# ugadiarov-la-phystech-edu/OCRL

Hardware: AMD Instinct MI355X
Metric: images/sec (node) SLATE pretrain 128x128, 6 slots, 3 iters (higher is better)
Workload: dtype f32

## Files before the change

### include/ocrl_hip.h

```cpp
#ifndef OCRL_HIP_H
#define OCRL_HIP_H
#include <stddef.h>

#ifdef __cplusplus
extern "C" {
#endif

#define OCRL_ABI_VERSION 5

const char* ocrl_last_error(void);
int ocrl_abi_version(void);

typedef struct ocrl_slate ocrl_slate;
typedef struct ocrl_slate_config {
    int obs_size, obs_channels;
    int vocab_size, d_model;
    int cnn_hidden;
    int num_slots, num_iterations, slot_size, mlp_hidden;
    int num_dec_blocks, num_dec_heads;
    float dropout;
    int max_batch;
    int use_bcdec;
    int hard;
    int num_slot_heads;
// ... 80 lines not shown
int ocrl_conv2d_bwd_weight_ex(const ocrl_conv_wgrad_desc* d, float* ws, size_t ws_floats, void* stream);
size_t ocrl_conv2d_first_fwd_ws_floats(void);
int ocrl_conv2d_first_fwd(const float* obs, const float* w, const float* bias, float* y, int B, int H, int W, int relu, float* ws, size_t ws_floats,
                          void* stream);
size_t ocrl_conv2d_first_wgrad_ws_floats(int B, int H, int W);
int ocrl_conv2d_first_bwd_weight(const float* obs, const float* dy, float* dw, float* db, int B, int H, int W, int accumulate, float* ws, size_t ws_floats,
                                 void* stream);
int ocrl_layernorm_fwd(const float* x, const float* gamma, const float* beta, float* y, float* mean, float* rstd, long long R, int F, void* stream);
int ocrl_layernorm_bwd(const float* dy, const float* x, const float* mean, const float* rstd, const float* gamma, float* dx, float* dgb,
                       long long R, int F, float* ws, size_t ws_floats, void* stream);

int ocrl_sa_input_plan(long long R, int out[3]);
int ocrl_sa_input_fwd(const float* e4, const float* gamma, const float* beta, const float* W0, const float* b0, const float* W2, const float* b2,
                      float* mean, float* rstd, float* h1, float* x, long long R, int max_wgs, void* stream);
int ocrl_sa_input_bwd(const float* dx, const float* h1, const float* e4, const float* mean, const float* rstd, const float* gamma, const float* beta,
                      const float* W0, const float* W2, float* de4, float* dW0, float* db0, float* dW2, float* db2, float* dgamma, float* dbeta,
                      long long R, int max_wgs, float* ws, size_t ws_floats, void* stream);

int ocrl_attention_fwd(const float* q, const float* k, const float* v, float* o, float* lse, int B, int T, int d, int h, int ld,
                       float p, unsigned long long seed, unsigned site, void* stream);
int ocrl_attention_bwd(const float* q, const float* k, const float* v, const float* o, const float* lse, const float* dO,
                       float* dq, float* dk, float* dv, float* delta, int B, int T, int d, int h, int ld,
                       float p, unsigned long long seed, unsigned site, void* stream);

typedef struct ocrl_xattn_desc {
    const float* x; const float* resid; const float* mem;
    const float* Wq; const float* Wk; const float* Wv; const float* Wo;
    float* ck; float* cv; float* Ab; float* AbT; float* Vo; float* VoT; float* y; float* P;
    const float* gd;
    float* Pd; float* dS; float* dx; float* dAb; float* dVo; float* dck; float* dcv; float* dWq; float* dWo;
    float* pq; float* po; float* cs_ws; size_t cs_ws_floats;
    int B, T, K, d, h;
    float p; unsigned long long seed; unsigned site_p, site_o;
} ocrl_xattn_desc;
size_t ocrl_xattn_desc_size(void);
int ocrl_xattn_plan(int K, int d, int h, int out[5]);
int ocrl_xattn_fwd(const ocrl_xattn_desc* d, void* stream);
int ocrl_xattn_bwd(const ocrl_xattn_desc* d, void* stream);
int ocrl_cross_attn_fwd(const float* Q, const float* Km, const float* Vm, float* O, float* P, int B, int T, int K, int d, int h, float p,
                        unsigned long long seed, unsigned site, void* stream);
size_t ocrl_cross_attn_bwd_ws_floats(int B, int T, int K, int d, int h);
int ocrl_cross_attn_bwd(const float* dO, const float* Q, const float* Km, const float* Vm, const float* P, float* dQ, float* dKm, float* dVm,
                        int B, int T, int K, int d, int h, float p, unsigned long long seed, unsigned site, float* ws, size_t ws_floats,
                        void* stream);

int ocrl_obs_u8_to_f32(const unsigned char* obs_hwc, float* obs_chw, int B, int H, int W, int C, void* stream);
// ... 216 lines not shown
```

### ocrl_amd/_lib.py

```python
import ctypes
import os
from ctypes import POINTER, c_char_p, c_float, c_int, c_longlong, c_size_t, c_uint, c_ulonglong, c_void_p

_HERE = os.path.dirname(os.path.abspath(__file__))
LIB_PATH = os.environ.get("OCRL_HIP_LIB") or os.path.join(_HERE, "libocrl_hip.so")
_lib = None


class SlateConfig(ctypes.Structure):
    _fields_ = [(n, c_int) for n in ("obs_size", "obs_channels", "vocab_size", "d_model", "cnn_hidden", "num_slots",
                                      "num_iterations", "slot_size", "mlp_hidden", "num_dec_blocks", "num_dec_heads")] + \
               [("dropout", c_float), ("max_batch", c_int), ("use_bcdec", c_int), ("hard", c_int), ("num_slot_heads", c_int)]


class IodineConfig(ctypes.Structure):
    _fields_ = [(n, c_int) for n in ("obs_size", "obs_channels", "slot_size", "num_iterations", "num_slots")] + \
               [("sigma", c_float), ("beta", c_float), ("layer_norm", c_int), ("ref_mlp_hidden", c_int), ("max_batch", c_int)]


class GemmDesc(ctypes.Structure):
    _fields_ = [("A", c_void_p), ("B", c_void_p), ("C", c_void_p)] + \
               [(n, c_int) for n in ("M", "N", "K", "lda", "ldb", "ldc", "akc", "bkc", "batch", "batch_inner")] + \
               [(n, c_longlong) for n in ("sA", "sB", "sC", "sAi", "sBi", "sCi")] + \
               [("splitk", c_int), ("alpha", c_float), ("bias", c_void_p), ("relu", c_int),
# ... 144 lines not shown
    L.ocrl_conv2d_wgrad_ws_floats.argtypes = [c_int, c_int, c_int, c_int, c_int]
    L.ocrl_conv2d_wgrad_ws_floats.restype = c_size_t
    L.ocrl_conv2d_bwd_weight.argtypes = [p, p, p, p, c_int, c_int, c_int, c_int, c_int, c_int, p, c_size_t, p]
    L.ocrl_conv_desc_size.restype = c_size_t
    L.ocrl_conv_wgrad_desc_size.restype = c_size_t
    for name, cls in (("ocrl_conv_desc", ConvDesc), ("ocrl_conv_wgrad_desc", ConvWgradDesc)):
        n = getattr(L, name + "_size")()
        if n != ctypes.sizeof(cls):
            raise RuntimeError(f"libocrl_hip.so: {name} is {n} bytes, this binding's {cls.__name__} {ctypes.sizeof(cls)}")
    L.ocrl_conv2d_ex.argtypes = [POINTER(ConvDesc), p, c_size_t, p]
    L.ocrl_conv2d_bwd_weight_ex.argtypes = [POINTER(ConvWgradDesc), p, c_size_t, p]
    L.ocrl_conv2d_first_fwd_ws_floats.restype = c_size_t
    L.ocrl_conv2d_first_fwd.argtypes = [p, p, p, p, c_int, c_int, c_int, c_int, p, c_size_t, p]
    L.ocrl_conv2d_first_wgrad_ws_floats.argtypes = [c_int, c_int, c_int]
    L.ocrl_conv2d_first_wgrad_ws_floats.restype = c_size_t
    L.ocrl_conv2d_first_bwd_weight.argtypes = [p, p, p, p, c_int, c_int, c_int, c_int, p, c_size_t, p]
    L.ocrl_layernorm_fwd.argtypes = [p, p, p, p, p, p, c_longlong, c_int, p]
    L.ocrl_layernorm_bwd.argtypes = [p, p, p, p, p, p, p, c_longlong, c_int, p, c_size_t, p]
    L.ocrl_sa_input_plan.argtypes = [c_longlong, POINTER(c_int * 3)]
    L.ocrl_sa_input_fwd.argtypes = [p] * 11 + [c_longlong, c_int, p]
    L.ocrl_sa_input_bwd.argtypes = [p] * 16 + [c_longlong, c_int, p, c_size_t, p]
    L.ocrl_attention_fwd.argtypes = [p, p, p, p, p, c_int, c_int, c_int, c_int, c_int, c_float, c_ulonglong, c_uint, p]
    L.ocrl_attention_bwd.argtypes = [p, p, p, p, p, p, p, p, p, p, c_int, c_int, c_int, c_int, c_int, c_float, c_ulonglong, c_uint, p]
    L.ocrl_xattn_desc_size.restype = c_size_t
    if L.ocrl_xattn_desc_size() != ctypes.sizeof(XattnDesc):
        raise RuntimeError(f"libocrl_hip.so: ocrl_xattn_desc is {L.ocrl_xattn_desc_size()} bytes, this binding's XattnDesc {ctypes.sizeof(XattnDesc)}")
    L.ocrl_xattn_plan.argtypes = [c_int, c_int, c_int, POINTER(c_int * 5)]
    L.ocrl_xattn_fwd.argtypes = [POINTER(XattnDesc), p]
    L.ocrl_xattn_bwd.argtypes = [POINTER(XattnDesc), p]
    L.ocrl_cross_attn_fwd.argtypes = [p, p, p, p, p, c_int, c_int, c_int, c_int, c_int, c_float, c_ulonglong, c_uint, p]
    L.ocrl_cross_attn_bwd_ws_floats.argtypes = [c_int] * 5
    L.ocrl_cross_attn_bwd_ws_floats.restype = c_size_t
    L.ocrl_cross_attn_bwd.argtypes = [p] * 8 + [c_int] * 5 + [c_float, c_ulonglong, c_uint, p, c_size_t, p]
    L.ocrl_obs_u8_to_f32.argtypes = [p, p, c_int, c_int, c_int, c_int, p]
    L.ocrl_prof_enable.argtypes = [c_uint]
    L.ocrl_prof_collect.argtypes = [POINTER(ctypes.c_double * 8), POINTER(c_longlong * 8), c_int]
    L.ocrl_iodine_create.argtypes = [POINTER(IodineConfig), POINTER(p)]
    L.ocrl_iodine_destroy.argtypes = [p]
    L.ocrl_iodine_destroy.restype = None
    L.ocrl_iodine_param_count.argtypes = [p]
    L.ocrl_iodine_param_info.argtypes = [p, c_int, c_char_p, c_int, POINTER(c_int * 4), POINTER(c_int), POINTER(c_longlong), POINTER(c_longlong)]
    L.ocrl_iodine_flat_size.argtypes = [p]
    L.ocrl_iodine_flat_size.restype = c_longlong
    L.ocrl_iodine_workspace_bytes.argtypes = [p]
    L.ocrl_iodine_workspace_bytes.restype = c_size_t
    L.ocrl_iodine_bind.argtypes = [p, p, p, p, p, p, c_size_t]
# ... 125 lines not shown
```

### ocrl_amd/csrc/attention.hip

```cpp
#include "common.h"
#include "kernels.h"
#include <stdlib.h>

#define FA_BLK 64
#ifndef FA_LPT
#define FA_LPT 1
#endif
#ifndef FA_BWD_WGS
#define FA_BWD_WGS 3
#endif

typedef float f32x4_t __attribute__((ext_vector_type(4)));

template <int DH>
struct FaCfg {
    static constexpr int NC = DH / 16;
    static constexpr int LD = DH + 4;
};

template <int DH>
__device__ inline void fa_load_tile(float* s, const float* __restrict__ g, long long bt0, int row0, int T, int d, int hoff, float scale) {
    constexpr int F4 = DH / 4;
    constexpr int LD = FaCfg<DH>::LD;
    for (int idx = threadIdx.x; idx < FA_BLK * F4; idx += 256) {
// ... 174 lines not shown
    __shared__ float part[256];
    const int F4 = d >> 2, RPB = 256 / F4, HF = F4 / h;
    const int rl = threadIdx.x / F4, c4 = threadIdx.x - rl * F4;
    const long long row = (long long)blockIdx.x * RPB + rl;
    float s = 0.f;
    if (rl < RPB && row < BT) {
        const float4 x = *reinterpret_cast<const float4*>(dO + row * d + c4 * 4), y = *reinterpret_cast<const float4*>(O + row * d + c4 * 4);
        s = x.x * y.x + x.y * y.y + x.z * y.z + x.w * y.w;
    }
    part[threadIdx.x] = s;
    __syncthreads();
    if ((int)threadIdx.x < RPB * h) {
        const int r2 = threadIdx.x / h, hd = threadIdx.x - r2 * h;
        const long long row2 = (long long)blockIdx.x * RPB + r2;
        if (row2 < BT) {
            float t = 0.f;
            for (int k = 0; k < HF; ++k) t += part[r2 * F4 + hd * HF + k];
            const long long bb = row2 / T, q = row2 % T;
            delta[(bb * h + hd) * T + q] = t;
        }
    }
}

template <int DH>
__global__ __launch_bounds__(256, FA_BWD_WGS) void attn_bwd_kv_kernel(AttnArgs p) {
    constexpr int NC = FaCfg<DH>::NC, LD = FaCfg<DH>::LD;
    __shared__ __attribute__((aligned(16))) float Qs[FA_BLK * LD];
    __shared__ __attribute__((aligned(16))) float Gs[FA_BLK * LD];
    __shared__ float Ls[FA_BLK], Ds[FA_BLK];
    const int nkb = (p.T + FA_BLK - 1) / FA_BLK;
    int bid = blockIdx.x;
    const int nbh = gridDim.x / nkb;
    const int kb = FA_LPT ? bid / nbh : fa_block_index(bid % nkb, bid / nkb, nkb);
    bid = FA_LPT ? bid % nbh : bid / nkb;
    const int hd = bid % p.h;
    const long long b = bid / p.h;
    const int T = p.T, T4 = attn_drop_ld(p.T), d = p.ld, hoff = hd * DH;
    const long long bt0 = b * T;
    const int lane = threadIdx.x & 63, wv = threadIdx.x >> 6;
    const int li = lane & 15, g = lane >> 4;
    const int k_abs = kb * FA_BLK + wv * 16 + li;
    const float scale = rsqrtf((float)DH);
    const long long bh = b * p.h + hd;

    float4 kf[NC], vf[NC];
#pragma unroll
    for (int c = 0; c < NC; ++c) {
        kf[c] = make_float4(0.f, 0.f, 0.f, 0.f);
        vf[c] = kf[c];
        if (k_abs < T) {
            kf[c] = *reinterpret_cast<const float4*>(p.k + (bt0 + k_abs) * d + hoff + 16 * c + 4 * g);
            vf[c] = *reinterpret_cast<const float4*>(p.v + (bt0 + k_abs) * d + hoff + 16 * c + 4 * g);
        }
    }
    f32x4_t dk[NC], dv[NC];
#pragma unroll
    for (int c = 0; c < NC; ++c) { dk[c] = (f32x4_t){0.f, 0.f, 0.f, 0.f}; dv[c] = dk[c]; }
    const uint32_t thr = drop_thresh(p.p);
    const float dsc = p.p > 0.f ? 1.0f / (1.0f - p.p) : 1.f;

    float4 rq[FaRegs<DH>::N], rg[FaRegs<DH>::N];
    float rl = 0.f, rd = 0.f;
    auto fetch = [&](int qt) {
        fa_fetch<DH>(rq, p.q, bt0, qt * FA_BLK, T, d, hoff);
        fa_fetch<DH>(rg, p.dO, bt0, qt * FA_BLK, T, p.d, hoff);
        if (threadIdx.x < FA_BLK) {
            const int qq = qt * FA_BLK + threadIdx.x;
            rl = qq < T ? p.lse[bh * T + qq] : 0.f;
            rd = qq < T ? p.delta[bh * T + qq] : 0.f;
        }
    };
    fetch(kb);
    for (int qt = kb; qt < nkb; ++qt) {
        __syncthreads();
        fa_commit<DH>(Qs, rq, scale);
        fa_commit<DH>(Gs, rg, 1.f);
        if (threadIdx.x < FA_BLK) { Ls[threadIdx.x] = rl; Ds[threadIdx.x] = rd; }
        __syncthreads();
        if (qt + 1 < nkb) fetch(qt + 1);
#pragma unroll
        for (int sq = 0; sq < 4; ++sq) {
            f32x4_t s = (f32x4_t){0.f, 0.f, 0.f, 0.f}, dp = s;
#pragma unroll
            for (int c = 0; c < NC; ++c) {
                const float4 a = *reinterpret_cast<const float4*>(Qs + (16 * sq + li) * LD + 16 * c + 4 * g);
                s = MFMA16(a.x, kf[c].x, s);
                s = MFMA16(a.y, kf[c].y, s);
                s = MFMA16(a.z, kf[c].z, s);
                s = MFMA16(a.w, kf[c].w, s);
                const float4 e = *reinterpret_cast<const float4*>(Gs + (16 * sq + li) * LD + 16 * c + 4 * g);
                dp = MFMA16(e.x, vf[c].x, dp);
                dp = MFMA16(e.y, vf[c].y, dp);
                dp = MFMA16(e.z, vf[c].z, dp);
                dp = MFMA16(e.w, vf[c].w, dp);
            }
            uint2 hb = make_uint2(0u, 0u);
            if (p.p > 0.f) {
                const int qh = qt * FA_BLK + 16 * sq + 4 * g + (li & 3);
                const uint64_t idx = ((uint64_t)bh * T + (uint64_t)(qh < T ? qh : 0)) * T4 + (uint64_t)(k_abs < T4 ? k_abs : 0);
                hb = rng_bits4(p.seed, p.site, idx >> 2);
            }
            uint2 hq[4];
            hq[0] = make_uint2(__builtin_amdgcn_update_dpp(0, (int)hb.x, 0x00, 0xF, 0xF, false), __builtin_amdgcn_update_dpp(0, (int)hb.y, 0x00, 0xF, 0xF, false));
            hq[1] = make_uint2(__builtin_amdgcn_update_dpp(0, (int)hb.x, 0x55, 0xF, 0xF, false), __builtin_amdgcn_update_dpp(0, (int)hb.y, 0x55, 0xF, 0xF, false));
            hq[2] = make_uint2(__builtin_amdgcn_update_dpp(0, (int)hb.x, 0xAA, 0xF, 0xF, false), __builtin_amdgcn_update_dpp(0, (int)hb.y, 0xAA, 0xF, 0xF, false));
            hq[3] = make_uint2(__builtin_amdgcn_update_dpp(0, (int)hb.x, 0xFF, 0xF, 0xF, false), __builtin_amdgcn_update_dpp(0, (int)hb.y, 0xFF, 0xF, 0xF, false));
            f32x4_t pd, ds;
#pragma unroll
            for (int r = 0; r < 4; ++r) {
                const int ql = 16 * sq + 4 * g + r;
                const int qa = qt * FA_BLK + ql;
                float pr = 0.f;
                if (qa < T && k_abs <= qa && k_abs < T) pr = __expf(s[r] - Ls[ql]);
                float keep = 1.f;
                if (p.p > 0.f) keep = rng_keep(hq[r], li & 3, thr) ? dsc : 0.f;
                pd[r] = pr * keep;
                ds[r] = pr * (dp[r] * keep - Ds[ql]);
            }
            float ag[4][NC], aq[4][NC];
#pragma unroll
            for (int r = 0; r < 4; ++r)
#pragma unroll
                for (int c = 0; c < NC; ++c) {
                    ag[r][c] = Gs[(16 * sq + 4 * g + r) * LD + 16 * c + li];
                    aq[r][c] = Qs[(16 * sq + 4 * g + r) * LD + 16 * c + li];
                }
            __builtin_amdgcn_sched_barrier(0);
#pragma unroll
            for (int r = 0; r < 4; ++r)
#pragma unroll
                for (int c = 0; c < NC; ++c) {
                    dv[c] = MFMA16(ag[r][c], pd[r], dv[c]);
                    dk[c] = MFMA16(aq[r][c], ds[r], dk[c]);
                }
        }
    }
    if (k_abs < T) {
#pragma unroll
        for (int c = 0; c < NC; ++c) {
            *reinterpret_cast<float4*>(p.dv + (bt0 + k_abs) * d + hoff + 16 * c + 4 * g) = make_float4(dv[c][0], dv[c][1], dv[c][2], dv[c][3]);
// ... 69 lines not shown
#pragma unroll
            for (int st = 0; st < 4; ++st) { sS[st] = MFMA16(a[st].y, qf[c].y, sS[st]); sP[st] = MFMA16(e[st].y, gf[c].y, sP[st]); }
#pragma unroll
            for (int st = 0; st < 4; ++st) { sS[st] = MFMA16(a[st].z, qf[c].z, sS[st]); sP[st] = MFMA16(e[st].z, gf[c].z, sP[st]); }
#pragma unroll
            for (int st = 0; st < 4; ++st) { sS[st] = MFMA16(a[st].w, qf[c].w, sS[st]); sP[st] = MFMA16(e[st].w, gf[c].w, sP[st]); }
        }
#pragma unroll
        for (int st = 0; st < 4; ++st) {
            const int key0 = kt * FA_BLK + 16 * st + 4 * g;
            uint2 bits = make_uint2(0u, 0u);
            if (p.p > 0.f) {
                const uint64_t idx = ((uint64_t)bh * T + (uint64_t)(q_abs < T ? q_abs : 0)) * T4 + (uint64_t)key0;
                bits = rng_bits4(p.seed, p.site, idx >> 2);
            }
#pragma unroll
            for (int r = 0; r < 4; ++r) {
                float pr = 0.f;
                if (q_abs < T && key0 + r <= q_abs && key0 + r < T) pr = __expf(sS[st][r] - lse);
                float keep = 1.f;
                if (p.p > 0.f) keep = rng_keep(bits, r, thr) ? dsc : 0.f;
                sS[st][r] = pr * (sP[st][r] * keep - dlt);
            }
        }
        float ak[2][4][NC];
#pragma unroll
        for (int r = 0; r < 4; ++r)
#pragma unroll
            for (int c = 0; c < NC; ++c) ak[0][r][c] = Ks[(4 * g + r) * LD + 16 * c + li];
#pragma unroll
        for (int st = 0; st < 4; ++st) {
            if (st + 1 < 4) {
#pragma unroll
                for (int r = 0; r < 4; ++r)
#pragma unroll
                    for (int c = 0; c < NC; ++c) ak[(st + 1) & 1][r][c] = Ks[(16 * (st + 1) + 4 * g + r) * LD + 16 * c + li];
            }
            __builtin_amdgcn_sched_barrier(0);
#pragma unroll
            for (int r = 0; r < 4; ++r)
#pragma unroll
                for (int c = 0; c < NC; ++c) dq[c] = MFMA16(ak[st & 1][r][c], sS[st][r], dq[c]);
            __builtin_amdgcn_sched_barrier(0);
        }
    }
    if (q_abs < T) {
// ... 160 lines not shown
                        dst[16 * c] = first ? v : dst[16 * c] + v;
                    }
                }
            }
        }
        if (k_abs < T) {
#pragma unroll
            for (int c = 0; c < NC; ++c) {
                *reinterpret_cast<float4*>(p.dv + (bt0 + k_abs) * d + hoff + 16 * c + 4 * g) = make_float4(dv[c][0], dv[c][1], dv[c][2], dv[c][3]);
                *reinterpret_cast<float4*>(p.dk + (bt0 + k_abs) * d + hoff + 16 * c + 4 * g) = make_float4(dk[c][0], dk[c][1], dk[c][2], dk[c][3]);
            }
        }
    }
}

template <int DH>
static int attn_launch_dh(const AttnArgs& a, int mode, hipStream_t st) {
    const int nblk = cdiv(a.T, FA_BLK);
    const dim3 grid(a.B * a.h * nblk), blk(256);
    if (mode == 0) {
        hipLaunchKernelGGL((attn_fwd_kernel<DH>), grid, blk, 0, st, a);
        OCRL_CHECK_LAUNCH("attn_fwd");
    } else {
        const long long BT = (long long)a.B * a.T;
        OCRL_REQUIRE(a.d % 4 == 0 && a.d <= 1024 && (a.d / 4) % a.h == 0, "attention: d must be a multiple of 4*h, <= 1024");
        hipLaunchKernelGGL(attn_delta_kernel, dim3(cdiv(BT, 256 / (a.d / 4))), dim3(256), 0, st, a.dO, a.o, a.delta, BT, a.T, a.d, a.h);
        OCRL_CHECK_LAUNCH("attn_delta");
        const char* fe = getenv("OCRL_ATTN_BWD");
        if (fe && atoi(fe) == 1) {
            hipLaunchKernelGGL((attn_bwd_fused_kernel<DH>), dim3(a.B * a.h), dim3(512), 0, st, a);
            OCRL_CHECK_LAUNCH("attn_bwd_fused");
        } else {
        hipLaunchKernelGGL((attn_bwd_kv_kernel<DH>), grid, blk, 0, st, a);
        OCRL_CHECK_LAUNCH("attn_bwd_kv");
        hipLaunchKernelGGL((attn_bwd_q_kernel<DH>), grid, blk, 0, st, a);
        OCRL_CHECK_LAUNCH("attn_bwd_q");
        }
    }
    return 0;
}

int attn_launch(const AttnArgs& a, int mode, hipStream_t st) {
    OCRL_REQUIRE(a.B > 0 && a.T > 0 && a.h > 0 && a.d % a.h == 0 && a.ld >= a.d && a.ld % 4 == 0, "attention: bad shape");
    OCRL_REQUIRE(a.q && a.k && a.v && a.o && a.lse, "attention: missing buffers");
    if (mode) OCRL_REQUIRE(a.dO && a.dq && a.dk && a.dv && a.delta, "attention backward: missing buffers");
    OCRL_REQUIRE((long long)a.T * a.T * a.B * a.h < (1ll << 62), "attention: too large");
    const int pi = prof_begin(mode ? PROF_ATTN_BWD : PROF_ATTN_FWD, st);
    int rc;
    switch (a.d / a.h) {
        case 16: rc = attn_launch_dh<16>(a, mode, st); break;
        case 32: rc = attn_launch_dh<32>(a, mode, st); break;
        case 48: rc = attn_launch_dh<48>(a, mode, st); break;
        case 64: rc = attn_launch_dh<64>(a, mode, st); break;
        default: ocrl_set_error("attention: head dim %d unsupported (16/32/48/64)", a.d / a.h); return 1;
    }
    prof_end(pi, st);
    return rc;
}
```

### ocrl_amd/csrc/capi.cpp

```cpp
#include <stdarg.h>
#include <stdint.h>
#include <string.h>

#include <new>

#include "../../include/ocrl_hip.h"
#include "iodine_model.h"
#include "slate_model.h"

static thread_local char g_err[512] = "";

void ocrl_set_error(const char* fmt, ...) {
    va_list ap;
    va_start(ap, fmt);
    vsnprintf(g_err, sizeof g_err, fmt, ap);
    va_end(ap);
}

template <class M>
struct Handle {
    using Model = M;
    M* m = nullptr;
};
struct ocrl_slate : Handle<SlateModel> {};
// ... 300 lines not shown
    return sa_input_fwd_launch(e4, gamma, beta, W0, b0, W2, b2, mean, rstd, nullptr, h1, x, R, max_wgs, ST(stream));
}
int ocrl_sa_input_bwd(const float* dx, const float* h1, const float* e4, const float* mean, const float* rstd, const float* gamma, const float* beta,
                      const float* W0, const float* W2, float* de4, float* dW0, float* db0, float* dW2, float* db2, float* dgamma, float* dbeta,
                      long long R, int max_wgs, float* ws, size_t ws_floats, void* stream) {
    return sa_input_bwd_launch(dx, h1, e4, mean, rstd, gamma, beta, W0, W2, de4, dW0, db0, dW2, db2, dgamma, dbeta, R, max_wgs, ws, ws_floats,
                               ST(stream));
}

int ocrl_attention_fwd(const float* q, const float* k, const float* v, float* o, float* lse, int B, int T, int d, int h, int ld, float p,
                       unsigned long long seed, unsigned site, void* stream) {
    AttnArgs a;
    a.q = q; a.k = k; a.v = v; a.o = o; a.lse = lse; a.B = B; a.T = T; a.d = d; a.h = h; a.ld = ld; a.p = p; a.seed = seed; a.site = site;
    return attn_launch(a, 0, ST(stream));
}
int ocrl_attention_bwd(const float* q, const float* k, const float* v, const float* o, const float* lse, const float* dO, float* dq,
                       float* dk, float* dv, float* delta, int B, int T, int d, int h, int ld, float p, unsigned long long seed,
                       unsigned site, void* stream) {
    AttnArgs a;
    a.q = q; a.k = k; a.v = v; a.o = const_cast<float*>(o); a.lse = const_cast<float*>(lse); a.B = B; a.T = T; a.d = d; a.h = h; a.ld = ld;
    a.p = p; a.seed = seed; a.site = site; a.dO = dO; a.dq = dq; a.dk = dk; a.dv = dv; a.delta = delta;
    return attn_launch(a, 1, ST(stream));
}

int ocrl_xattn_plan(int K, int d, int h, int out[5]) {
    if (!out) { ocrl_set_error("ocrl_xattn_plan: null argument"); return 1; }
    XaPlan p;
    if (!xattn_plan(K, d, h, &p)) ocrl_set_error("ocrl_xattn_plan: no folded form for K %d, d %d, heads %d", K, d, h);
    out[0] = p.supported ? 1 : 0; out[1] = p.KP; out[2] = p.NC; out[3] = p.NM; out[4] = (int)p.lds;
    return 0;
}
size_t ocrl_xattn_desc_size(void) { return sizeof(ocrl_xattn_desc); }
static XaHost xattn_host(const ocrl_xattn_desc& d) {
    XaHost hx;
    hx.x = d.x; hx.P = d.P; hx.Ab = d.Ab; hx.AbT = d.AbT; hx.Vo = d.Vo; hx.VoT = d.VoT;
    hx.B = d.B; hx.T = d.T; hx.K = d.K; hx.d = d.d; hx.h = d.h; hx.p = d.p; hx.seed = d.seed; hx.site_p = d.site_p; hx.site_o = d.site_o;
    return hx;
}
int ocrl_xattn_fwd(const ocrl_xattn_desc* d, void* stream) {
    if (!d) { ocrl_set_error("ocrl_xattn_fwd: null descriptor"); return 1; }
    if (!xattn_supported(d->K, d->d, d->h)) { ocrl_set_error("ocrl_xattn_fwd: no folded form for K %d, d %d, heads %d", d->K, d->d, d->h); return 1; }
    if (d->B < 1 || d->T < 1 || !d->x || !d->resid || !d->mem || !d->Wq || !d->Wk || !d->Wv || !d->Wo || !d->ck || !d->cv || !d->Ab || !d->AbT ||
        !d->Vo || !d->VoT || !d->y || !d->P) {
        ocrl_set_error("ocrl_xattn_fwd: null buffer or empty shape");
        return 1;
    }
// ... 79 lines not shown
```

### ocrl_amd/csrc/kernels.h

```cpp
#pragma once
#include "common.h"
#include "../../include/ocrl_hip.h"

enum { PROF_CONV5 = 0, PROF_CONV_OTHER = 1, PROF_WGRAD = 2, PROF_GEMM = 3, PROF_SA_FWD = 4, PROF_SA_BWD = 5, PROF_ATTN_FWD = 6, PROF_ATTN_BWD = 7, PROF_NTAGS = 8 };
int prof_begin(int tag, hipStream_t st);
void prof_end(int idx, hipStream_t st);

struct GemmArgs {
    const float* A = nullptr;
    const float* B = nullptr;
    float* C = nullptr;
    int M = 0, N = 0, K = 0;
    int lda = 0, ldb = 0, ldc = 0;
    int akc = 1, bkc = 1;
    int batch = 1;
    int batch_inner = 1;
    long long sA = 0, sB = 0, sC = 0;
    long long sAi = 0, sBi = 0, sCi = 0;
    int splitk = 1;
    long long sCsplit = 0;
    float alpha = 1.f;
    const float* bias = nullptr;
    int relu = 0;
    float drop_p = 0.f;
// ... 370 lines not shown
                           hipStream_t st);
int multi_clip_rmsprop_launch(FlatSegs t, float* norm, float clip, float lr, double alpha, double eps, float* ws, size_t ws_floats, hipStream_t st);
int store_u64_launch(unsigned long long* dst, unsigned long long v, hipStream_t st);
int slot_init_launch(const float* mu, const float* logsig, const float* noise, float* slots0, int BK, int D, unsigned long long seed, hipStream_t st,
                     const unsigned long long* seed_dev = nullptr);
int slot_init_bwd_launch(const float* dslots0, const float* logsig, const float* noise, float* dmu, float* dlogsig, int BK, int D, unsigned long long seed, hipStream_t st);
int copy_launch(const float* src, float* dst, long long n, hipStream_t st);
int argmax_pos_launch(const float* pred, int* tokens, int B, int T, int V, int t, hipStream_t st, int dense_rows = 0);
int embed_step_launch(const int* tokens, const float* dict, const float* bos, const float* pe, float* out, int B, int T, int d, int t, hipStream_t st);
int decode_attn_launch(const float* qkv, float* out, int B, int T, int t, int d, int h, int ld, hipStream_t st);
int onehot_launch(const int* tokens, float* z, long long rows, int V, hipStream_t st);

struct AttnArgs {
    const float *q = nullptr, *k = nullptr, *v = nullptr;
    float* o = nullptr;
    float* lse = nullptr;
    int B = 0, T = 0, d = 0, h = 0;
    int ld = 0;
    float p = 0.f;
    unsigned long long seed = 0;
    unsigned site = 0;
    const float* dO = nullptr;
    float *dq = nullptr, *dk = nullptr, *dv = nullptr, *delta = nullptr;
};
int attn_launch(const AttnArgs& a, int mode, hipStream_t st);

enum { BCAST_L1_RELU = 0, BCAST_L1_ELU = 1 };
int bcast_l1_class_sum_launch(const float* in, float* out, long long BK, int ks, int forward, hipStream_t st);
int bcast_l1_fwd_launch(const float* P1, const float* T, const float* bias, float* c1, long long BK, int S, int ks, int act, hipStream_t st);
size_t bcast_l1_bwd_ws_floats(long long BK, int S, int ks);
int bcast_l1_bwd_launch(const float* g, float* dT, long long BK, int S, int ks, float* ws, size_t ws_floats, hipStream_t st);
int bc_posconv_launch(const float* Wc, float* P1, int S, hipStream_t st);
int bc_posconv_bwd_launch(const float* G, float* dWc, int S, hipStream_t st);
int io_p1_launch(const float* Wxy, const float* b1, float* P1, int S, hipStream_t st);
int io_w1_grad_launch(const float* dW1r, const float* G, float* dW1, float* db1, int S, int L, hipStream_t st);

int bc_compose_launch(const float* W1, const float* Wpos, const float* bpos, float* Wc, float* W1r, int D, hipStream_t st);
int bc_compose_bwd_launch(const float* W1, const float* Wpos, const float* bpos, const float* dWc, const float* dW1r, float* dW1,
                          float* dWpos, float* dbpos, int D, hipStream_t st);
int bc_c4_pack_launch(const float* W, float* Wk, float* Wb, int co_n, hipStream_t st);
int bc_c4_fwd_launch(const float* X, const float* Wk, const float* bias4, float* Y, int Bn, int S, hipStream_t st);
int bc_c4_bwd_data_launch(const float* dY, const float* Wb, const float* act, float* dX, int Bn, int S, hipStream_t st, int elu = 0);
int bc_c4_wgrad_blocks(int Bn, int S);
int bc_c4_wgrad_launch(const float* X, const float* dY, float* part, int Bn, int S, hipStream_t st);
int bc_mix_launch(const float* out4, const float* obs, float* recon, float* dout4, float* loss_out, int B, int K, int S, int C, float* ws,
                  size_t ws_floats, hipStream_t st);

int io_sample_launch(const float* mu, const float* ls, const float* noise, float* eps_out, float* slots, float* kl_out, long long n,
// ... 23 lines not shown
```

### ocrl_amd/csrc/slate_model.cpp

```cpp
#include "slate_model.h"

#include <stdlib.h>

#include <math.h>
#include <stdarg.h>
#include <string.h>

static std::string fmt(const char* f, ...) {
    char buf[256];
    va_list ap;
    va_start(ap, f);
    vsnprintf(buf, sizeof buf, f, ap);
    va_end(ap);
    return buf;
}

SlateModel::SlateModel(const SlateConfig& c) : cfg(c) {
    S = c.obs_size; E = S / 4; T = E * E; N = S * S; V = c.vocab; d = c.d_model; C = c.cnn_hidden;
    K = c.num_slots; I = c.num_iters; D = c.slot_size; H = c.mlp_hidden; NB = c.num_blocks; NH = c.num_heads;
    DH = d / NH; Bmax = c.max_batch; SH = c.slot_heads > 0 ? c.slot_heads : 1;
    const int ch = c.obs_channels;
    add_param("_dvae._encoder.0.m.weight", {64, ch, 4, 4}, 0); add_param("_dvae._encoder.0.m.bias", {64}, 0);
    for (int i = 1; i < 7; ++i) { add_param(fmt("_dvae._encoder.%d.m.weight", i), {64, 64, 1, 1}, 0); add_param(fmt("_dvae._encoder.%d.m.bias", i), {64}, 0); }
    add_param("_dvae._encoder.7.weight", {V, 64, 1, 1}, 0); add_param("_dvae._encoder.7.bias", {V}, 0);
// ... 201 lines not shown
        k.ln1 = carve(nullptr, BT * d); k.ln1_mean = carve(nullptr, BT); k.ln1_rstd = carve(nullptr, BT);
        k.q = carve(nullptr, BT * 3 * d); k.k = k.q + d; k.v = k.q + 2 * d;
        k.lse = carve(nullptr, B * NH * (size_t)T); k.ao = carve(nullptr, BT * d); k.x1 = carve(nullptr, BT * d);
        k.ln2 = carve(nullptr, BT * d); k.ln2_mean = carve(nullptr, BT); k.ln2_rstd = carve(nullptr, BT);
        k.cq = carve(nullptr, BT * d); k.ck = carve(nullptr, BK * d); k.cv = carve(nullptr, BK * d);
        k.cP = carve(nullptr, B * NH * (size_t)T * K); k.cao = carve(nullptr, BT * d); k.x2 = carve(nullptr, BT * d);
        k.ln3 = carve(nullptr, BT * d); k.ln3_mean = carve(nullptr, BT); k.ln3_rstd = carve(nullptr, BT);
        k.f1 = carve(fmt("blk%d.ffn_hidden", b).c_str(), BT * 4 * d); k.x3 = carve(nullptr, BT * d);
    }
    bg_.resize(NB);
    {
        const size_t NC = xattn_supported(K, d, NH) ? (size_t)NH * xattn_kp(K, NH) : 16;
        xa_zero_base_ = carve_pos();
        for (int b = 0; b < NB; ++b) {
            Blk& k = blk_[b];
            k.xaAb = carve(nullptr, B * NC * d); k.xaAbT = carve(nullptr, B * NC * d); k.xaVo = carve(nullptr, B * NC * d); k.xaVoT = carve(nullptr, B * NC * d);
        }
        xa_zero_floats_ = (size_t)(carve_pos() - xa_zero_base_);
        for (int b = 0; b < NB; ++b) { bg_[b].xaPd = carve(nullptr, BT * NC); bg_[b].xaDs = carve(nullptr, BT * NC); }
        xa_dAb_ = carve(nullptr, B * NC * d); xa_dVo_ = carve(nullptr, B * NC * d);
        xa_pq_ = carve(nullptr, B * (size_t)d * d); xa_po_ = carve(nullptr, B * (size_t)d * d);
    }
    attn_delta_ = carve(nullptr, B * NH * (size_t)T);
    lnf_ = carve("dec_out", BT * d); lnf_mean_ = carve(nullptr, BT); lnf_rstd_ = carve(nullptr, BT);
    pred_ = carve("pred", BT * V);
    gx_ = carve(nullptr, BT * d); gbr_ = carve(nullptr, BT * d); gt1_ = carve(nullptr, BT * d); gt2_ = carve(nullptr, BT * d);
    gt3_ = carve(nullptr, BT * d); gf1_ = carve(nullptr, BT * 4 * d); gqkv_ = carve(nullptr, BT * 3 * d);
    for (int b = 0; b < NB; ++b) {
        BlkG& q = bg_[b];
        if (b == 0) { q.gbr[0] = gbr_; q.gf1 = gf1_; q.gt2 = gt2_; q.gqkv = gqkv_; }
        else { q.gbr[0] = carve(nullptr, BT * d); q.gf1 = carve(nullptr, BT * 4 * d); q.gt2 = carve(nullptr, BT * d); q.gqkv = carve(nullptr, BT * 3 * d); }
        q.gbr[1] = carve(nullptr, BT * d); q.gbr[2] = carve(nullptr, BT * d);
    }
    scratch3_ = carve(nullptr, scratch_floats_);
    gmem_ = carve(nullptr, BK * d); gck_ = carve(nullptr, BK * d); gcv_ = carve(nullptr, BK * d);
    gdA_ = carve(nullptr, BN * 64); gdB_ = carve(nullptr, BN * 64);
    }
    col0_ = dw0p_ = nullptr;
    if (!first_direct()) {
        const int ldc0 = (25 * cfg.obs_channels + 3) & ~3;
        col0_ = carve(nullptr, BN * ldc0); dw0p_ = carve(nullptr, (size_t)64 * ldc0);
    }
    end_layout();
}

int SlateModel::bind(float* p, float* g, float* m, float* v, void* ws, size_t ws_bytes) {
    RC(check_buffers(p, g, ws, ws_bytes));
// ... 481 lines not shown
        } else {
        RC(lin_bwd_x(gd, d, P(bw.co), gt1_, d, BT, d, d, nullptr, 0, nullptr, 0, L));
        RC(cross_attn_bwd_launch(gt1_, k.cq, k.ck, k.cv, k.cP, q.gt2, gck_, gcv_, B, T, K, d, NH, p, last_.seed, site + 2, L.scratch, L.scratch_floats, L));
        RC(after(W, L, ring_event()));
        RC(lin_bwd_w(gd_co, d, k.cao, d, G(bw.co), nullptr, BT, d, d, 1.f, W));
        RC(lin_bwd_w(q.gt2, d, k.ln2, d, G(bw.cq), nullptr, BT, d, d, 1.f, W));
        RC(lin_bwd_x(q.gt2, d, P(bw.cq), gt1_, d, BT, d, d, nullptr, 0, nullptr, 0, L));
        }
        {
            const Lane& X = xattn_ ? W : L;
            RC(lin_bwd_w(gck_, d, mem_, d, G(bw.ck), nullptr, BK, d, d, 1.f, X));
            RC(lin_bwd_w(gcv_, d, mem_, d, G(bw.cv), nullptr, BK, d, d, 1.f, X));
            RC(lin_bwd_x(gck_, d, P(bw.ck), gmem_, d, BK, d, d, nullptr, 0, gmem_, d, X));
            RC(lin_bwd_x(gcv_, d, P(bw.cv), gmem_, d, BK, d, d, nullptr, 0, gmem_, d, X));
        }
        RC(layernorm_bwd_launch(gt1_, k.x1, k.ln2_mean, k.ln2_rstd, P(bw.ln2.w), gx_,
                                G(bw.ln2.w), BT, d, 1, 0, L.scratch, L.scratch_floats, L));
        RC(drop_gx(site + 1, q.gbr[2]));
        const float* gd_o = gd;
        RC(lin_bwd_x(gd, d, P(bw.o), gt1_, d, BT, d, d, nullptr, 0, nullptr, 0, L));
        {
            AttnArgs a = self_attn_args(b);
            a.dO = gt1_; a.dq = q.gqkv; a.dk = q.gqkv + d; a.dv = q.gqkv + 2 * d; a.delta = attn_delta_;
            RC(attn_launch(a, 1, L));
        }
        RC(after(W, L, ring_event()));
        RC(lin_bwd_w(gd_o, d, k.ao, d, G(bw.o), nullptr, BT, d, d, 1.f, W));
        RC(lin_bwd_w(q.gqkv, 3 * d, k.ln1, d, G(bw.qkv), nullptr, BT, 3 * d, d, 1.f, W));
        RC(lin_bwd_x(q.gqkv, 3 * d, P(bw.qkv), gt1_, d, BT, 3 * d, d, nullptr, 0, nullptr, 0, L));
        if (b == 0) {
            RC(axpy_launch(gx_, gt1_, BT * d, 1.f, L));
            RC(layernorm_bwd_launch(gt1_, xin, k.ln1_mean, k.ln1_rstd, P(bw.ln1.w), gx_,
                                    G(bw.ln1.w), BT, d, 0, 0, L.scratch, L.scratch_floats, L));
        } else {
            RC(layernorm_bwd_launch(gt1_, xin, k.ln1_mean, k.ln1_rstd, P(bw.ln1.w), gx_,
                                    G(bw.ln1.w), BT, d, 1, 0, L.scratch, L.scratch_floats, L));
        }
    }
    RC(embed_bwd_launch(gx_, tokens_, G(w_.dict), B, T, V, d, p, last_.seed, L.scratch, L.scratch_floats, L));
    RC(fill_launch(G(w_.pe), (long long)(T + 1) * d, 0.f, L));
    RC(colsum_launch(gx_, (long long)T * d, G(w_.pe), B, T * d, 0, 1.f, L.scratch, L.scratch_floats, L));
    RC(copy_launch(G(w_.pe), G(w_.bos), d, L));
    if (xattn_) RC(after(L, W, ring_event()));
    RC(lin_bwd_w(gmem_, d, slots_, D, G(w_.slotproj), nullptr, BK, d, D, 1.f, L));
    RC(lin_bwd_x(gmem_, d, P(w_.slotproj), gslots_, D, BK, d, D, nullptr, 0, nullptr, 0, L));
    return 0;
// ... 252 lines not shown
```

### ocrl_amd/csrc/slate_model.h

```cpp
#pragma once
#include <map>
#include <string>
#include <vector>

#include "kernels.h"
#include "model_base.h"
#include "slot_attn_host.h"

struct SlateConfig {
    int obs_size = 64, obs_channels = 3, vocab = 4096, d_model = 192, cnn_hidden = 64;
    int num_slots = 5, num_iters = 3, slot_size = 192, mlp_hidden = 192;
    int num_blocks = 4, num_heads = 4;
    float dropout = 0.1f;
    int max_batch = 1;
    int use_bcdec = 0;
    int hard = 0;
    int slot_heads = 1;
};

struct StepInputs {
    const float* obs = nullptr;
    int B = 0;
    float tau = 1.f;
    int train = 1;
// ... 126 lines not shown
        float *xaAb, *xaAbT, *xaVo, *xaVoT;
    };
    int sa_input_ = 1;
    bool xattn_ = false;
    float *xa_dAb_ = nullptr, *xa_dVo_ = nullptr, *xa_pq_ = nullptr, *xa_po_ = nullptr;
    size_t xa_zero_floats_ = 0;
    float* xa_zero_base_ = nullptr;
    std::vector<Blk> blk_;
    struct BlkG { float *gbr[3], *gf1, *gt2, *gqkv, *xaPd, *xaDs; };
    std::vector<BlkG> bg_;
    struct EncGraph { hipGraphExec_t exec = nullptr; int warm = 0; };
    std::map<int, EncGraph> enc_graphs_;
    int enc_graph_mode_ = -1;
    hipStream_t cap_ = nullptr;
    float* obs_stage_ = nullptr;
    unsigned long long* seed_dev_ = nullptr;
    int dw_mode_ = 0;
    hipStream_t side2_ = nullptr;
    float* scratch3_ = nullptr;
    hipEvent_t ev_dw_[8] = {nullptr, nullptr, nullptr, nullptr, nullptr, nullptr, nullptr, nullptr};
    hipEvent_t ev_join2_ = nullptr;
    int ev_dw_next_ = 0;
    float *attn_delta_;
    float *lnf_, *lnf_mean_, *lnf_rstd_, *pred_;
    float *gqkv_;
    float *gx_, *gbr_, *gt1_, *gt2_, *gt3_, *gf1_, *gmem_, *gck_, *gcv_, *gslots_, *gslots0_;
    float *gA_, *gB_, *gC_;
    float *gdA_, *gdB_;
    float *gmap_;
    float *col0_, *dw0p_;
    float* obs_keep_ = nullptr;
    bool first_direct() const { return cfg.obs_channels == 3; }
    float *bc_Wc_, *bc_W1r_, *bc_P1_, *bc_M_, *bc_T_, *bc_c1_, *bc_c2_, *bc_c3_, *bc_out4_, *bc_dout4_, *bc_gA_, *bc_gB_;
    float *bc_pk_[2], *bc_pkb_[2], *bc_Wk4_, *bc_Wb4_, *bc_dW1r_, *bc_dWc_, *bc_dT_, *bc_dM_, *bc_G1_;
};
```

Before: 1758.

## Hand off dS from KV backward kernel to new dQ kernel via workspace

The attention backward KV kernel now writes its computed dS tiles to a triangular workspace, and a new dQ kernel reads them back instead of recomputing QK^T, softmax, dropout and dP. The batch is chunked to fit a configurable workspace capacity, 2 GiB by default. This trades recomputation FLOPs for extra global memory traffic and workspace.

```diff
diff --git a/include/ocrl_hip.h b/include/ocrl_hip.h
--- a/include/ocrl_hip.h
+++ b/include/ocrl_hip.h
@@ -126,6 +126,10 @@
 int ocrl_attention_bwd(const float* q, const float* k, const float* v, const float* o, const float* lse, const float* dO,
                        float* dq, float* dk, float* dv, float* delta, int B, int T, int d, int h, int ld,
                        float p, unsigned long long seed, unsigned site, void* stream);
+size_t ocrl_attention_bwd_ds_floats(int B, int T, int h);
+int ocrl_attention_bwd_ws(const float* q, const float* k, const float* v, const float* o, const float* lse, const float* dO,
+                          float* dq, float* dk, float* dv, float* delta, int B, int T, int d, int h, int ld,
+                          float p, unsigned long long seed, unsigned site, float* ds, size_t ds_floats, void* stream);
 
 typedef struct ocrl_xattn_desc {
     const float* x; const float* resid; const float* mem;
diff --git a/ocrl_amd/_lib.py b/ocrl_amd/_lib.py
--- a/ocrl_amd/_lib.py
+++ b/ocrl_amd/_lib.py
@@ -190,6 +190,9 @@
     L.ocrl_sa_input_bwd.argtypes = [p] * 16 + [c_longlong, c_int, p, c_size_t, p]
     L.ocrl_attention_fwd.argtypes = [p, p, p, p, p, c_int, c_int, c_int, c_int, c_int, c_float, c_ulonglong, c_uint, p]
     L.ocrl_attention_bwd.argtypes = [p, p, p, p, p, p, p, p, p, p, c_int, c_int, c_int, c_int, c_int, c_float, c_ulonglong, c_uint, p]
+    L.ocrl_attention_bwd_ds_floats.argtypes = [c_int, c_int, c_int]
+    L.ocrl_attention_bwd_ds_floats.restype = c_size_t
+    L.ocrl_attention_bwd_ws.argtypes = L.ocrl_attention_bwd.argtypes[:-1] + [p, c_size_t, p]
     L.ocrl_xattn_desc_size.restype = c_size_t
     if L.ocrl_xattn_desc_size() != ctypes.sizeof(XattnDesc):
         raise RuntimeError(f"libocrl_hip.so: ocrl_xattn_desc is {L.ocrl_xattn_desc_size()} bytes, this binding's XattnDesc {ctypes.sizeof(XattnDesc)}")
diff --git a/ocrl_amd/csrc/attention.hip b/ocrl_amd/csrc/attention.hip
--- a/ocrl_amd/csrc/attention.hip
+++ b/ocrl_amd/csrc/attention.hip
@@ -220,7 +220,10 @@
     }
 }
 
-template <int DH>
+#define FA_DS_TILE (FA_BLK * FA_BLK)
+__host__ __device__ inline size_t fa_ds_tiles(int nblk) { return (size_t)nblk * (nblk + 1) / 2; }
+
+template <int DH, bool HANDOFF>
 __global__ __launch_bounds__(256, FA_BWD_WGS) void attn_bwd_kv_kernel(AttnArgs p) {
     constexpr int NC = FaCfg<DH>::NC, LD = FaCfg<DH>::LD;
     __shared__ __attribute__((aligned(16))) float Qs[FA_BLK * LD];
@@ -232,7 +235,7 @@
     const int kb = FA_LPT ? bid / nbh : fa_block_index(bid % nkb, bid / nkb, nkb);
     bid = FA_LPT ? bid % nbh : bid / nkb;
     const int hd = bid % p.h;
-    const long long b = bid / p.h;
+    const long long b = p.b0 + bid / p.h;
     const int T = p.T, T4 = attn_drop_ld(p.T), d = p.ld, hoff = hd * DH;
     const long long bt0 = b * T;
     const int lane = threadIdx.x & 63, wv = threadIdx.x >> 6;
@@ -240,6 +243,7 @@
     const int k_abs = kb * FA_BLK + wv * 16 + li;
     const float scale = rsqrtf((float)DH);
     const long long bh = b * p.h + hd;
+    float* const dsw = HANDOFF ? p.ds + ((size_t)bid * fa_ds_tiles(nkb) + kb) * FA_DS_TILE + 4 * g * FA_BLK + wv * 16 + li : nullptr;
 
     float4 kf[NC], vf[NC];
 #pragma unroll
@@ -276,6 +280,7 @@
         if (threadIdx.x < FA_BLK) { Ls[threadIdx.x] = rl; Ds[threadIdx.x] = rd; }
         __syncthreads();
         if (qt + 1 < nkb) fetch(qt + 1);
+        float* const dst = HANDOFF ? dsw + fa_ds_tiles(qt) * FA_DS_TILE : nullptr;
 #pragma unroll
         for (int sq = 0; sq < 4; ++sq) {
             f32x4_t s = (f32x4_t){0.f, 0.f, 0.f, 0.f}, dp = s;
@@ -314,6 +319,7 @@
                 if (p.p > 0.f) keep = rng_keep(hq[r], li & 3, thr) ? dsc : 0.f;
                 pd[r] = pr * keep;
                 ds[r] = pr * (dp[r] * keep - Ds[ql]);
+                if (HANDOFF) dst[(16 * sq + r) * FA_BLK] = ds[r];
             }
             float ag[4][NC], aq[4][NC];
 #pragma unroll
@@ -429,6 +435,74 @@
                 if (p.p > 0.f) keep = rng_keep(bits, r, thr) ? dsc : 0.f;
                 sS[st][r] = pr * (sP[st][r] * keep - dlt);
             }
+        }
+        float ak[2][4][NC];
+#pragma unroll
+        for (int r = 0; r < 4; ++r)
+#pragma unroll
+            for (int c = 0; c < NC; ++c) ak[0][r][c] = Ks[(4 * g + r) * LD + 16 * c + li];
+#pragma unroll
+        for (int st = 0; st < 4; ++st) {
+            if (st + 1 < 4) {
+#pragma unroll
+                for (int r = 0; r < 4; ++r)
+#pragma unroll
+                    for (int c = 0; c < NC; ++c) ak[(st + 1) & 1][r][c] = Ks[(16 * (st + 1) + 4 * g + r) * LD + 16 * c + li];
+            }
+            __builtin_amdgcn_sched_barrier(0);
+#pragma unroll
+            for (int r = 0; r < 4; ++r)
+#pragma unroll
+                for (int c = 0; c < NC; ++c) dq[c] = MFMA16(ak[st & 1][r][c], sS[st][r], dq[c]);
+            __builtin_amdgcn_sched_barrier(0);
+        }
+    }
+    if (q_abs < T) {
+#pragma unroll
+        for (int c = 0; c < NC; ++c)
+            *reinterpret_cast<float4*>(p.dq + (bt0 + q_abs) * d + hoff + 16 * c + 4 * g) =
+                make_float4(dq[c][0] * scale, dq[c][1] * scale, dq[c][2] * scale, dq[c][3] * scale);
+    }
+}
+
+template <int DH>
+__global__ __launch_bounds__(256, 4) void attn_bwd_dq_kernel(AttnArgs p) {
+    constexpr int NC = FaCfg<DH>::NC, LD = FaCfg<DH>::LD;
+    __shared__ __attribute__((aligned(16))) float Ks[FA_BLK * LD];
+    const int nqb = (p.T + FA_BLK - 1) / FA_BLK;
+    int bid = blockIdx.x;
+    const int nbh = gridDim.x / nqb;
+    const int qb = FA_LPT ? nqb - 1 - bid / nbh : fa_block_index(bid % nqb, bid / nqb, nqb);
+    bid = FA_LPT ? bid % nbh : bid / nqb;
+    const int hd = bid % p.h;
+    const long long b = p.b0 + bid / p.h;
+    const int T = p.T, d = p.ld, hoff = hd * DH;
+    const long long bt0 = b * T;
+    const int lane = threadIdx.x & 63, wv = threadIdx.x >> 6;
+    const int li = lane & 15, g = lane >> 4;
+    const int q_abs = qb * FA_BLK + wv * 16 + li;
+    const float scale = rsqrtf((float)DH);
+    const float* const dsr = p.ds + ((size_t)bid * fa_ds_tiles(nqb) + fa_ds_tiles(qb)) * FA_DS_TILE + (wv * 16 + li) * FA_BLK + 4 * g;
+
+    f32x4_t dq[NC];
+#pragma unroll
+    for (int c = 0; c < NC; ++c) dq[c] = (f32x4_t){0.f, 0.f, 0.f, 0.f};
+    float4 rk[FaRegs<DH>::N];
+    f32x4_t rs[4];
+    fa_fetch<DH>(rk, p.k, bt0, 0, T, d, hoff);
+#pragma unroll
+    for (int st = 0; st < 4; ++st) rs[st] = *reinterpret_cast<const f32x4_t*>(dsr + 16 * st);
+    for (int kt = 0; kt <= qb; ++kt) {
+        __syncthreads();
+        fa_commit<DH>(Ks, rk, 1.f);
+        __syncthreads();
+        f32x4_t sS[4];
+#pragma unroll
+        for (int st = 0; st < 4; ++st) sS[st] = rs[st];
+        if (kt < qb) {
+            fa_fetch<DH>(rk, p.k, bt0, (kt + 1) * FA_BLK, T, d, hoff);
+#pragma unroll
+            for (int st = 0; st < 4; ++st) rs[st] = *reinterpret_cast<const f32x4_t*>(dsr + (size_t)(kt + 1) * FA_DS_TILE + 16 * st);
         }
         float ak[2][4][NC];
 #pragma unroll
@@ -635,22 +709,49 @@
         hipLaunchKernelGGL((attn_fwd_kernel<DH>), grid, blk, 0, st, a);
         OCRL_CHECK_LAUNCH("attn_fwd");
     } else {
+        OCRL_REQUIRE(a.d % 4 == 0 && a.d <= 1024 && (a.d / 4) % a.h == 0, "attention: d must be a multiple of 4*h, <= 1024");
+        const char* fe = getenv("OCRL_ATTN_BWD");
+        const int form = fe ? atoi(fe) : 0;
+        const size_t per_image = attn_bwd_ds_floats(1, a.T, a.h);
+        const size_t room = (a.ds && form != 1 && form != 2) ? a.ds_floats / per_image : 0;
+        if (room >= 1) {
+            OCRL_REQUIRE(((uintptr_t)a.ds & 15) == 0, "attention backward: the dS workspace must be 16-byte aligned");
+            const int chunk = room < (size_t)a.B ? (int)room : a.B;
+            for (int b0 = 0; b0 < a.B; b0 += chunk) {
+                const int nb = a.B - b0 < chunk ? a.B - b0 : chunk;
+                const long long r0 = (long long)b0 * a.T, rows = (long long)nb * a.T;
+                hipLaunchKernelGGL(attn_delta_kernel, dim3(cdiv(rows, 256 / (a.d / 4))), dim3(256), 0, st, a.dO + r0 * a.d, a.o + r0 * a.d,
+                                   a.delta + r0 * a.h, rows, a.T, a.d, a.h);
+                OCRL_CHECK_LAUNCH("attn_delta");
+                AttnArgs c = a;
+                c.b0 = b0;
+                const dim3 cgrid(nb * a.h * nblk);
+                hipLaunchKernelGGL((attn_bwd_kv_kernel<DH, true>), cgrid, blk, 0, st, c);
+                OCRL_CHECK_LAUNCH("attn_bwd_kv");
+                hipLaunchKernelGGL((attn_bwd_dq_kernel<DH>), cgrid, blk, 0, st, c);
+                OCRL_CHECK_LAUNCH("attn_bwd_dq");
+            }
+            return 0;
+        }
         const long long BT = (long long)a.B * a.T;
-        OCRL_REQUIRE(a.d % 4 == 0 && a.d <= 1024 && (a.d / 4) % a.h == 0, "attention: d must be a multiple of 4*h, <= 1024");
         hipLaunchKernelGGL(attn_delta_kernel, dim3(cdiv(BT, 256 / (a.d / 4))), dim3(256), 0, st, a.dO, a.o, a.delta, BT, a.T, a.d, a.h);
         OCRL_CHECK_LAUNCH("attn_delta");
-        const char* fe = getenv("OCRL_ATTN_BWD");
-        if (fe && atoi(fe) == 1) {
+        if (form == 1) {
             hipLaunchKernelGGL((attn_bwd_fused_kernel<DH>), dim3(a.B * a.h), dim3(512), 0, st, a);
             OCRL_CHECK_LAUNCH("attn_bwd_fused");
         } else {
-        hipLaunchKernelGGL((attn_bwd_kv_kernel<DH>), grid, blk, 0, st, a);
-        OCRL_CHECK_LAUNCH("attn_bwd_kv");
-        hipLaunchKernelGGL((attn_bwd_q_kernel<DH>), grid, blk, 0, st, a);
-        OCRL_CHECK_LAUNCH("attn_bwd_q");
+            hipLaunchKernelGGL((attn_bwd_kv_kernel<DH, false>), grid, blk, 0, st, a);
+            OCRL_CHECK_LAUNCH("attn_bwd_kv");
+            hipLaunchKernelGGL((attn_bwd_q_kernel<DH>), grid, blk, 0, st, a);
+            OCRL_CHECK_LAUNCH("attn_bwd_q");
         }
     }
     return 0;
+}
+
+size_t attn_bwd_ds_floats(int B, int T, int h) {
+    if (B <= 0 || T <= 0 || h <= 0) return 0;
+    return (size_t)B * h * fa_ds_tiles(cdiv(T, FA_BLK)) * FA_DS_TILE;
 }
 
 int attn_launch(const AttnArgs& a, int mode, hipStream_t st) {
diff --git a/ocrl_amd/csrc/capi.cpp b/ocrl_amd/csrc/capi.cpp
--- a/ocrl_amd/csrc/capi.cpp
+++ b/ocrl_amd/csrc/capi.cpp
@@ -346,6 +346,15 @@
     a.p = p; a.seed = seed; a.site = site; a.dO = dO; a.dq = dq; a.dk = dk; a.dv = dv; a.delta = delta;
     return attn_launch(a, 1, ST(stream));
 }
+size_t ocrl_attention_bwd_ds_floats(int B, int T, int h) { return attn_bwd_ds_floats(B, T, h); }
+int ocrl_attention_bwd_ws(const float* q, const float* k, const float* v, const float* o, const float* lse, const float* dO, float* dq,
+                          float* dk, float* dv, float* delta, int B, int T, int d, int h, int ld, float p, unsigned long long seed,
+                          unsigned site, float* ds, size_t ds_floats, void* stream) {
+    AttnArgs a;
+    a.q = q; a.k = k; a.v = v; a.o = const_cast<float*>(o); a.lse = const_cast<float*>(lse); a.B = B; a.T = T; a.d = d; a.h = h; a.ld = ld;
+    a.p = p; a.seed = seed; a.site = site; a.dO = dO; a.dq = dq; a.dk = dk; a.dv = dv; a.delta = delta; a.ds = ds; a.ds_floats = ds_floats;
+    return attn_launch(a, 1, ST(stream));
+}
 
 int ocrl_xattn_plan(int K, int d, int h, int out[5]) {
     if (!out) { ocrl_set_error("ocrl_xattn_plan: null argument"); return 1; }
diff --git a/ocrl_amd/csrc/kernels.h b/ocrl_amd/csrc/kernels.h
--- a/ocrl_amd/csrc/kernels.h
+++ b/ocrl_amd/csrc/kernels.h
@@ -416,8 +416,12 @@
     unsigned site = 0;
     const float* dO = nullptr;
     float *dq = nullptr, *dk = nullptr, *dv = nullptr, *delta = nullptr;
+    float* ds = nullptr;
+    size_t ds_floats = 0;
+    int b0 = 0;
 };
 int attn_launch(const AttnArgs& a, int mode, hipStream_t st);
+size_t attn_bwd_ds_floats(int B, int T, int h);
 
 enum { BCAST_L1_RELU = 0, BCAST_L1_ELU = 1 };
 int bcast_l1_class_sum_launch(const float* in, float* out, long long BK, int ks, int forward, hipStream_t st);
diff --git a/ocrl_amd/csrc/slate_model.cpp b/ocrl_amd/csrc/slate_model.cpp
--- a/ocrl_amd/csrc/slate_model.cpp
+++ b/ocrl_amd/csrc/slate_model.cpp
@@ -247,7 +247,19 @@
         xa_pq_ = carve(nullptr, B * (size_t)d * d); xa_po_ = carve(nullptr, B * (size_t)d * d);
     }
     attn_delta_ = carve(nullptr, B * NH * (size_t)T);
-    lnf_ = carve("dec_out", BT * d); lnf_mean_ = carve(nullptr, BT); lnf_rstd_ = carve(nullptr, BT);
+    {
+        if (attn_ds_cap_ < 0) {
+            const char* fe = getenv("OCRL_ATTN_BWD");
+            const char* mb = getenv("OCRL_ATTN_DS_MB");
+            const int form = fe ? atoi(fe) : 0;
+            const long long mbs = mb ? atoll(mb) : 2048;
+            attn_ds_cap_ = (form == 1 || form == 2 || mbs < 0) ? 0 : mbs * (1ll << 20) / (long long)sizeof(float);
+        }
+        const size_t cap = (size_t)attn_ds_cap_, full = attn_bwd_ds_floats((int)B, T, NH);
+        attn_ds_floats_ = full < cap ? full : cap;
+        attn_ds_ = attn_ds_floats_ ? carve(nullptr, attn_ds_floats_) : nullptr;
+    }
+    lnf_ =carve("dec_out", BT * d); lnf_mean_ = carve(nullptr, BT); lnf_rstd_ = carve(nullptr, BT);
     pred_ = carve("pred", BT * V);
     gx_ = carve(nullptr, BT * d); gbr_ = carve(nullptr, BT * d); gt1_ = carve(nullptr, BT * d); gt2_ = carve(nullptr, BT * d);
     gt3_ = carve(nullptr, BT * d); gf1_ = carve(nullptr, BT * 4 * d); gqkv_ = carve(nullptr, BT * 3 * d);
@@ -775,6 +787,7 @@
         {
             AttnArgs a = self_attn_args(b);
             a.dO = gt1_; a.dq = q.gqkv; a.dk = q.gqkv + d; a.dv = q.gqkv + 2 * d; a.delta = attn_delta_;
+            a.ds = attn_ds_; a.ds_floats = attn_ds_floats_;
             RC(attn_launch(a, 1, L));
         }
         RC(after(W, L, ring_event()));
diff --git a/ocrl_amd/csrc/slate_model.h b/ocrl_amd/csrc/slate_model.h
--- a/ocrl_amd/csrc/slate_model.h
+++ b/ocrl_amd/csrc/slate_model.h
@@ -172,6 +172,9 @@
     hipEvent_t ev_join2_ = nullptr;
     int ev_dw_next_ = 0;
     float *attn_delta_;
+    float *attn_ds_ = nullptr;
+    size_t attn_ds_floats_ = 0;
+    long long attn_ds_cap_ = -1;
     float *lnf_, *lnf_mean_, *lnf_rstd_, *pred_;
     float *gqkv_;
     float *gx_, *gbr_, *gt1_, *gt2_, *gt3_, *gf1_, *gmem_, *gck_, *gcv_, *gslots_, *gslots0_;
```

Result: faster. 1808, median of 6 (+2.9%).
